# tspooner/rl_markets

Measured on AMD Instinct MI355X. Metric: env-steps/sec (whole node) at 65 536 parallel books, higher is better.
Workload: dtype f64

## Files before the change

rl_markets_amd/csrc/lob_engine.hip:

```cpp
#define LOB_TU_SPLIT 1
#define LOB_TU_MAIN 1
#include <hip/hip_runtime.h>
#include <math.h>
#include <stdio.h>
#include <stdlib.h>
#include <string.h>

#include <algorithm>
#include <climits>
#include <initializer_list>
#include <string>
#include <vector>

#include "lob_internal.h"
#include "lob_fast.h"
#include "lob_kernels.h"
#include "lob_launch.h"

#include "lob_engine_impl.h"

namespace {

void make_rndseq(uint32_t* t) {
    const int total = 344 + 4 * 2048;
// ... 114 lines not shown
            float ms = 0;
            hipEventElapsedTime(&ms, pr.first, pr.second);
            kv.second.total_ms += ms;
            kv.second.launches++;
            e->event_pool.push_back(pr.first);
            e->event_pool.push_back(pr.second);
        }
        kv.second.pending.clear();
    }
}

int device_error_rc(i32 flag) {
    if (flag) {
        std::string m = "device reported a condition on which the reference throws:";
        if (flag & LOB_ERR_BAD_ORDER_PRICE) m += " [order price <= 0]";
        if (flag & LOB_ERR_BAD_LEVEL) m += " [level price/volume <= 0]";
        if (flag & LOB_ERR_UNDEF_PRICE) m += " [undefined book price]";
        if (flag & LOB_ERR_TRADE_OVERFLOW) m += " [more trade price levels in one event than max_trades]";
        if (flag & LOB_ERR_TRACK_UNDERRUN) m += " [market-track ring underrun: raise LOB_TRACK_RING or lower LOB_TRACK_REFILL]";
        lob_set_error(m);
        return LOB_EDATA;
    }
    return LOB_OK;
}
int check_device_errors(lob_engine* e) {
    i32 flag = 0;
    HIPCHK(hipMemcpyAsync(&flag, e->S.error_flag, sizeof flag, hipMemcpyDeviceToHost, e->stream));
    HIPCHK(hipStreamSynchronize(e->stream));
    return device_error_rc(flag);
}

int finalize_episode(lob_engine* e) {
    if (!e->episode_open) return LOB_OK;
    lobk_finalize(e->stream, e->P.T <= 2, (const DevParams*)e->P_dev, e->S);
    HIPCHK(hipGetLastError());
    HIPCHK(hipStreamSynchronize(e->stream));
    e->episode_open = false;
    return LOB_OK;
}

void launch_env(lob_engine* e, hipStream_t st, const i32* actions, int count_updates, int b0, int nb, int par) {
    lobk_env(st, e->plan.env_lanes, e->P.T <= 2, (const DevParams*)e->P_dev, e->S, actions, count_updates, b0, nb, e->step_id, par);
}
void maybe_refill_track(lob_engine* e) {
    if (!e->chunked || ++e->steps_since_fill < e->sw.track_refill) return;
    e->steps_since_fill = 0;
    TimedLaunch t(e, "prepass_extend_kernel", nullptr, true);
    lobk_prepass_extend(e->stream, e->P.T <= 2, e->sw.prepass_roles, (const DevParams*)e->P_dev, e->S);
}
void launch_memo(lob_engine* e, int par, int which, int reset_lpar) {
    TimedLaunch t(e, "memo_kernel");
    hipLaunchKernelGGL(memo_kernel, dim3(256), dim3(256), 0, e->stream, e->P, e->S, (const uint32_t*)e->rnd_dev, par, which, (u64)e->theta_ver, reset_lpar);
}

void launch_step_log(lob_engine* e) {
    if (!e->slog_armed) return;
    TimedLaunch t(e, "step_log_kernel");
    StepLogSrc s;
    s.done = e->S.done; s.time_ms = e->S.time_ms; s.rec_cur = e->S.rec_cur; s.last_action = e->S.last_action;
    s.ask_level = e->S.ask_level; s.bid_level = e->S.bid_level; s.total_ticks = e->S.total_ticks;
    s.position = e->S.position;
    s.ask_quote = e->S.ask_quote; s.bid_quote = e->S.bid_quote; s.pnl_step = e->S.pnl_step;
    s.ep_pnl = e->S.ep_pnl; s.ep_bandh = e->S.ep_bandh; s.ep_reward = e->S.ep_reward;
    s.records = e->S.records; s.rec_phase = e->S.rec_phase;
    s.n_events = e->S.n_events; s.Wd = e->P.Wd; s.w_ask0 = drec_ask_px(e->P.D, e->P.T); s.w_bid0 = drec_bid_px(e->P.D, e->P.T);
    s.sel = e->slog_sel; s.n_sel = e->slog_n; s.cap = e->slog_cap;
    s.rows = e->slog_rows; s.n_rows = e->slog_cnt; s.n_lost = e->slog_cnt + e->slog_n;
    lobk_step_log(e->stream, s);
}
// ... 122 lines not shown
    P.epi_epoch = 0;
    P.seed = p->seed; P.book_id_offset = p->book_id_offset;
    P.exp_learn_first = e->sw.exp_learn_first ? 1 : 0;

    DevState& S = e->S;
    memset(&S, 0, sizeof S);
    const size_t B = (size_t)n_books;
    S.B = n_books; S.D = P.D; S.T = P.T; S.W = P.W;
    int rc = LOB_OK;
    auto alloc = [&](auto* ptr, size_t count) { if (rc == LOB_OK) rc = dev_alloc(e, ptr, count); };
#define X(t, n) alloc(&S.n, B);
    LOB_ENV_FIELDS(X)
#undef X
    alloc(&S.hdr, B);
    auto alloc_rm = [&](RMPtrs& r, int w) {
        r.w = w;
        alloc(&r.ring, B * w); alloc(&r.cnt, B); alloc(&r.head, B); alloc(&r.sum, B); alloc(&r.mean, B); alloc(&r.s, B);
    };
    auto alloc_acc = [&](AccPtrs& r, int w) {
        r.w = w;
        alloc(&r.ring, B * w); alloc(&r.cnt, B); alloc(&r.head, B); alloc(&r.sum, B);
    };
    alloc_rm(S.f_midprice, p->lb_mpm);
    alloc_rm(S.f_volatility, p->lb_vlt);
    alloc_rm(S.f_ask_tx, p->lb_svl);
    alloc_rm(S.f_bid_tx, p->lb_svl);
    alloc_rm(S.spread_window, p->lb_spread);
    alloc_rm(S.pnl_ups, p->lb_pnl);
    alloc_rm(S.pnl_downs, p->lb_pnl);
    alloc_rm(S.tp_mp, p->lb_target);
    alloc_acc(S.f_vwap_numer, p->lb_vwap);
    alloc_acc(S.f_vwap_denom, p->lb_vwap);
    alloc(&S.meta, B); alloc(&S.prep, B); alloc(&S.ewma_up, B); alloc(&S.ewma_down, B); alloc(&S.tp_val, B); alloc(&S.persist, B * LOB_PERSIST_N);
    alloc(&S.k_stop, B); alloc(&S.vars, B * 3 * 16); alloc(&S.qs_last, B * LOB_N_ACTIONS); alloc(&S.tr_idx, B * (size_t)P.trace_gens * 32);
    alloc(&S.tr_alive, B * (size_t)P.trace_gens); alloc(&S.theta, (size_t)P.M * (P.theta_private ? B : 1));
    alloc(&S.theta_nz, LOB_NZ_NWORDS(P.M) * (P.theta_private ? B : 1));
    if (P.algo == LOB_ALGO_DOUBLE_Q) {
        alloc(&S.theta_b, (size_t)P.M * (P.theta_private ? B : 1)); alloc(&S.theta_b_nz, LOB_NZ_NWORDS(P.M) * (P.theta_private ? B : 1));
        alloc(&S.qs_last_b, B * LOB_N_ACTIONS); alloc(&S.mt_state, B * LOB_MT_N); alloc(&S.mt_idx, B);
    }
    {
        const bool rl = P.r_learn != 0;
        const size_t nr = rl ? (P.theta_private ? B : 1) : 1;
        alloc(&S.rho, nr); alloc(&S.rho_inc, nr); alloc(&S.rho_cnt, nr); alloc(&S.rl_t, rl ? B : 1);
    }
    alloc(&S.tr_sig, B * (size_t)P.trace_gens * 4); alloc(&S.tr_cbslot, B * (size_t)P.trace_gens);
    {
        int slots = 2048;
        while ((size_t)slots < 8 * B && slots < (1 << 22)) slots <<= 1;
        if (e->sw.cb_slots) slots = e->sw.cb_slots;
        S.cb_slots = slots;
        alloc(&S.cb_key, (size_t)slots); alloc(&S.cb_ident, (size_t)slots * 8);
        S.cb_reps = e->sw.acc_reps ? e->sw.acc_reps : P.memo ? 8 : 1;
        alloc(&S.cb_acc, (size_t)S.cb_reps * slots * 2); alloc(&S.cb_touch, (size_t)slots); alloc(&S.cb_list, 2 * (size_t)slots);
        S.cb_segs = std::min(2048, slots / 4);
        alloc(&S.cb_count, 2 * (size_t)S.cb_segs);
        if (rc == LOB_OK && hipMemsetAsync(S.cb_key, 0xff, (size_t)slots * 8, e->stream) != hipSuccess) rc = LOB_EHIP;
        if (e->plan.dense_ids) {
            alloc(&S.cb_dense, (size_t)slots); alloc(&S.cb_free, (size_t)LOB_CBD_CAP); alloc(&S.cb_free_n, 16);
            alloc(&S.tr_cbd, B * (size_t)P.trace_gens); alloc(&S.cb_part, (size_t)LOB_ACD_MAX_BLOCKS * LOB_CBD_CAP);
            alloc(&S.cb_red, (size_t)LOB_ACD_GROUPS * LOB_CBD_CAP);
            if (rc == LOB_OK && hipMemsetAsync(S.cb_dense, 0xff, (size_t)slots * 4, e->stream) != hipSuccess) rc = LOB_EHIP;
            if (rc == LOB_OK && hipMemsetAsync(S.tr_cbd, 0xff, B * (size_t)P.trace_gens * 8, e->stream) != hipSuccess) rc = LOB_EHIP;
            if (rc == LOB_OK) {
                std::vector<i32> fl(LOB_CBD_CAP), fn(16);
                const int per = LOB_CBD_CAP / 8;
                int have = per;
// ... 1105 lines not shown
```

rl_markets_amd/csrc/lob_engine_impl.h:

```cpp
#ifndef LOB_ENGINE_IMPL_H
#define LOB_ENGINE_IMPL_H

#include <hip/hip_runtime.h>
#include <string.h>

#include <map>
#include <string>
#include <thread>
#include <utility>
#include <vector>

#include "lob_internal.h"
#include "lob_kernels.h"
#include "lob_launch.h"
#include "lob_devbuf.h"

#define HIPCHK(expr)                                                                         \
    do {                                                                                     \
        hipError_t _e = (expr);                                                              \
        if (_e != hipSuccess) {                                                              \
            lob_set_error(std::string(#expr) + ": " + hipGetErrorString(_e));                \
            return LOB_EHIP;                                                                 \
        }                                                                                    \
    } while (0)
// ... 42 lines not shown
    int groups = 1;
    bool combine = false, memo = false, carry_verdicts = false, sarsa_lanes = false;
    bool q_lanes = false;
    bool q_pair = false;
    bool t_light = false;
    bool fuse = false;
    bool fused_act_ok = false;
    bool env_step = false, half_waves = false, env16 = false;
    bool inline_ok = false;
    int env_lanes = 64;
    bool acc_block_ok = false;
    bool dense_ids = false;
    bool acc_fuse_ok = false;
    bool rest_side_ok = false;
    bool learn_first = false;
};

struct lob_engine {
    int device = 0;
    int B = 0;
    lob_params params;
    Switches sw;
    EnginePlan plan;
    DevParams P;
    DevParams* P_dev = nullptr;
    DevState S;
    DevState* S_dev = nullptr;
    DevState S_pushed;
    hipStream_t stream = nullptr;
    hipStream_t stream2 = nullptr;
    hipEvent_t ev_fork = nullptr, ev_join = nullptr, ev_stagger = nullptr;
    hipEvent_t ev_rest_go = nullptr, ev_rest_done = nullptr;
    long long flow[8] = {0, 0, 0, 0, 0, 0, 0, 0};
    long long hint_reads = 0, hint_misses = 0;
    bool dense_ever = false;
    u64* rest_hint = nullptr;
    u64* rest_hint_dev = nullptr;
    hipEvent_t hint_ev[LOB_HINT_RING] = {};
    long long hint_step = 0;
    unsigned long long hint_serial = 0;
    uint32_t hint_tags[LOB_HINT_RING] = {};
    int hint_now = 0;
    int rest_recent = 0;
    int reg_apar = 0;
    int td_parity = 0;
    int step_id = 0;
    int list_par = 0;
    int last_par = 0;
    int n_cus = 256;
    bool chunked = false;
    int steps_since_fill = 0;
    uint64_t theta_ver = 1;
    bool half_open = false;
    bool hits_ok = false;
    int steps_on_lists = 0;
    std::vector<void*> allocs;
    lob::DevBuf<uint32_t> spx_gather;
    int spx_world = 0;
    uint32_t* spx_union = nullptr;
    i32* spx_block_cnt = nullptr;
    i64* spx_block_off = nullptr;
    i64* spx_total = nullptr;
    f64* spx_buf = nullptr;
    int64_t spx_cap = 0, spx_count = 0;
    i64* spx_total_host = nullptr;
    hipEvent_t spx_ev = nullptr;
// ... 150 lines not shown
```

rl_markets_amd/csrc/lob_env.h:

```cpp
#ifndef LOB_ENV_H
#define LOB_ENV_H

#include <hip/hip_runtime.h>

#include "lob_internal.h"
#include "lob_state.h"

LOB_HD int drec_pad4(int n) { return (n + 3) & ~3; }
LOB_HD int drec_words(int D, int T) { return 4 + 4 * drec_pad4(D) + drec_pad4(2 * T); }
LOB_HD int drec_ask_px(int, int) { return 4; }
LOB_HD int drec_ask_vol(int D, int) { return 4 + drec_pad4(D); }
LOB_HD int drec_bid_px(int D, int) { return 4 + 2 * drec_pad4(D); }
LOB_HD int drec_bid_vol(int D, int) { return 4 + 3 * drec_pad4(D); }
LOB_HD int drec_trades(int D, int) { return 4 + 4 * drec_pad4(D); }
LOB_HD void drec_from_abi(const uint32_t* src, int D, int T, uint32_t* dst) {
    const int Wd = drec_words(D, T);
    for (int i = 0; i < Wd; i++) dst[i] = 0;
    dst[0] = src[LOB_REC_TIME];
    dst[1] = src[LOB_REC_FLAGS];
    for (int l = 0; l < D; l++) {
        dst[drec_ask_px(D, T) + l] = src[lob_rec_ask_px(D, T) + l];
        dst[drec_ask_vol(D, T) + l] = src[lob_rec_ask_vol(D, T) + l];
        dst[drec_bid_px(D, T) + l] = src[lob_rec_bid_px(D, T) + l];
        dst[drec_bid_vol(D, T) + l] = src[lob_rec_bid_vol(D, T) + l];
// ... 1462 lines not shown
            const f64 lm = (m.lap0 + m.lbp0) / 2.0;
            valid = ((m.ap0 - m.bp0) >= 0.0) && (mp > 0.0) && (fabs(mp - lm) < mp);
        }
        if (valid) break;
    }
    return true;
}

__device__ inline void persist_io(const DevState& S, int b, bool save) {
    int i = 0;
    const int B = S.B;
#define X(n)                                                                                   \
    if (save) { S.persist[(size_t)(i + 0) * B + b] = S.n.sum[b]; S.persist[(size_t)(i + 1) * B + b] = S.n.mean[b]; S.persist[(size_t)(i + 2) * B + b] = S.n.s[b]; } \
    else { S.n.sum[b] = S.persist[(size_t)(i + 0) * B + b]; S.n.mean[b] = S.persist[(size_t)(i + 1) * B + b]; S.n.s[b] = S.persist[(size_t)(i + 2) * B + b]; }   \
    i += 3;
    X(f_midprice) X(f_volatility) X(f_ask_tx) X(f_bid_tx) X(spread_window) X(tp_mp)
#undef X
#define X(n)                                                            \
    if (save) S.persist[(size_t)i * B + b] = S.n.sum[b];                \
    else S.n.sum[b] = S.persist[(size_t)i * B + b];                     \
    i += 1;
    X(f_vwap_numer) X(f_vwap_denom)
#undef X
    if (save) {
        S.persist[(size_t)(i + 0) * B + b] = S.ewma_up[b];
        S.persist[(size_t)(i + 1) * B + b] = S.ewma_down[b];
        S.persist[(size_t)(i + 2) * B + b] = S.tp_val[b];
    } else {
        S.ewma_up[b] = S.persist[(size_t)(i + 0) * B + b];
        S.ewma_down[b] = S.persist[(size_t)(i + 1) * B + b];
        S.tp_val[b] = S.persist[(size_t)(i + 2) * B + b];
    }
}

__device__ inline void prepass_begin(const EnvCtx& c, PrepState& st, BookMeta& M) {
    const DevParams& P = c.P;
    const DevState& S = c.S;
    const int b = c.b;
    MarketR m;
    m.cursor = 0; m.time_ms = 0; m.rec_cur = -1; m.rec_last = -1;
    m.ap0 = m.bp0 = m.lap0 = m.lbp0 = 0.0;
    m.a_tv = m.b_tv = 0;
    m.a_obsval = m.b_obsval = 0.0; m.a_obsvol = m.b_obsvol = 0;
    m.ewma_up = S.ewma_up[b]; m.ewma_down = S.ewma_down[b]; m.tp_val = S.tp_val[b];
    m.records = 0;
#define X(n) S.n.cnt[b] = 0;
    LOB_ROLLING_MEANS(X)
    LOB_ACCUMULATORS(X)
#undef X
    M.n_track = 0; M.k_warm = -1; M.init_ok = 0; M.complete = 0; M._pad = 0;
    M.ex_first = -1; M.ex_cur = -1; M.ex_last = -1; M.ex_time = 0; M.ex_records = 0;
    bool ok = true;
    while (ok && !is_open(P, m.time_ms)) ok = mk_update_book_profiles(c, m);
    M.rec_cur0 = m.rec_cur; M.rec_last0 = m.rec_last; M.time0 = m.time_ms;
    M.mid0 = (m.ap0 + m.bp0) / 2.0; M.mid_prev0 = (m.lap0 + m.lbp0) / 2.0;
    if (!ok) { M.ex_cur = m.rec_cur; M.ex_last = m.rec_last; M.ex_time = m.time_ms; M.complete = 1; }
    st.cursor = m.cursor; st.time_ms = m.time_ms; st.rec_cur = m.rec_cur; st.rec_last = m.rec_last;
    st.ap0 = m.ap0; st.bp0 = m.bp0; st.lap0 = m.lap0; st.lbp0 = m.lbp0;
    st.a_tv = m.a_tv; st.b_tv = m.b_tv;
    st.ewma_up = m.ewma_up; st.ewma_down = m.ewma_down; st.tp_val = m.tp_val;
    st.records = m.records;
    st.k = 0;
    st.prev_first = m.rec_cur;
}

__device__ inline void prepass_begin_books(const EnvCtx& c, PrepState& st, BookMeta& M) {
    const DevParams& P = c.P;
    MarketR m;
    m.cursor = 0; m.time_ms = 0; m.rec_cur = -1; m.rec_last = -1;
    m.ap0 = m.bp0 = m.lap0 = m.lbp0 = 0.0;
    m.a_tv = m.b_tv = 0;
    m.a_obsval = m.b_obsval = 0.0; m.a_obsvol = m.b_obsvol = 0;
    m.ewma_up = m.ewma_down = m.tp_val = 0.0;
    m.records = 0;
    M.n_track = 0; M.k_warm = -1; M.init_ok = 0; M.complete = 0; M._pad = 0;
    M.ex_first = -1; M.ex_cur = -1; M.ex_last = -1; M.ex_time = 0; M.ex_records = 0;
    bool ok = true;
    while (ok && !is_open(P, m.time_ms)) ok = mk_update_book_profiles(c, m);
    M.rec_cur0 = m.rec_cur; M.rec_last0 = m.rec_last; M.time0 = m.time_ms;
    M.mid0 = (m.ap0 + m.bp0) / 2.0; M.mid_prev0 = (m.lap0 + m.lbp0) / 2.0;
    if (!ok) { M.ex_cur = m.rec_cur; M.ex_last = m.rec_last; M.ex_time = m.time_ms; M.complete = 1; }
    st.cursor = m.cursor; st.time_ms = m.time_ms; st.rec_cur = m.rec_cur; st.rec_last = m.rec_last;
    st.ap0 = m.ap0; st.bp0 = m.bp0; st.lap0 = m.lap0; st.lbp0 = m.lbp0;
    st.a_tv = m.a_tv; st.b_tv = m.b_tv;
    st.ewma_up = st.ewma_down = st.tp_val = 0.0;
    st.records = m.records;
    st.k = 0;
    st.prev_first = m.rec_cur;
}

template <int TM>
__device__ inline void prepass_run(const EnvCtx& c, PrepState& st, BookMeta& M, int k_stop, bool write_track) {
    const DevParams& P = c.P;
    const DevState& S = c.S;
    const int b = c.b, B = S.B;
    MarketR m;
    m.cursor = st.cursor; m.time_ms = st.time_ms; m.rec_cur = st.rec_cur; m.rec_last = st.rec_last;
    m.ap0 = st.ap0; m.bp0 = st.bp0; m.lap0 = st.lap0; m.lbp0 = st.lbp0;
    m.a_tv = st.a_tv; m.b_tv = st.b_tv;
    m.a_obsval = m.b_obsval = 0.0; m.a_obsvol = m.b_obsvol = 0;
    m.ewma_up = st.ewma_up; m.ewma_down = st.ewma_down; m.tp_val = st.tp_val;
    m.records = st.records;
    int k = st.k;
    int prev_first = st.prev_first;
    RMReg w_mid, w_vol, w_spr, w_tp, w_atx, w_btx;
    AccReg w_vn, w_vd;
    rm_load(S.f_midprice, b, w_mid); rm_load(S.f_volatility, b, w_vol); rm_load(S.spread_window, b, w_spr);
    rm_load(S.tp_mp, b, w_tp); rm_load(S.f_ask_tx, b, w_atx); rm_load(S.f_bid_tx, b, w_btx);
    acc_load(S.f_vwap_numer, b, w_vn); acc_load(S.f_vwap_denom, b, w_vd);
#ifndef LOB_PRE_TOUCH
#define LOB_PRE_TOUCH 0
#endif
#if LOB_PRE_TOUCH
    PreRow<TM> R0;
    uint32_t nt[4] = {0u, 0u, 0u, 0u};
#else
    PreRow<TM> R0, R1;
#endif
    i32 t1 = 0, t2 = 0;
    bool piped = false;
    int band_px = 0, band_tk = 0;
    rm_prep(S.f_midprice, B, b, w_mid); rm_prep(S.f_volatility, B, b, w_vol); rm_prep(S.spread_window, B, b, w_spr);
    rm_prep(S.tp_mp, B, b, w_tp); rm_prep(S.f_ask_tx, B, b, w_atx); rm_prep(S.f_bid_tx, B, b, w_btx);
// ... 109 lines not shown
            }
            {
                f64 v_a = (f64)m.a_tv, v_b = (f64)m.b_tv;
                t.mv[LOB_MV_IMB] = (f32)((v_a + v_b) > 0 ? 5 * (v_b - v_a) / (v_b + v_a) : 0.0);
                f64 q_a = w_atx.sum, q_b = w_btx.sum;
                t.mv[LOB_MV_SVL] = (f32)((q_a + q_b) > 0 ? 5 * (q_b - q_a) / (q_a + q_b) : 0.0);
            }
            {
                f64 var = w_vol.s / (f64)(w_vol.cnt - 1);
                f64 sd = var > 0 ? sqrt(var) : 0.0;
                t.mv[LOB_MV_VOL] = (f32)ulb(5.0 * sd, 0.0, 10.0);
                f64 u = m.ewma_up, d = m.ewma_down;
                t.mv[LOB_MV_RSI] = (f32)((u + d) != 0.0 ? 5.0 * (u - d) / (u + d) : 0.0);
                f64 vw = w_vn.sum / w_vd.sum;
                t.mv[LOB_MV_VWAP] = (f32)ulb(vw / w_spr.mean, -10.0, 10.0);
                t.mv[7] = 0.0f;
            }
            c.track_w(k) = t;
            if (M.k_warm < 0 && w_atx.cnt == S.f_ask_tx.w && w_btx.cnt == S.f_bid_tx.w && w_vn.cnt == S.f_vwap_numer.w &&
                w_vd.cnt == S.f_vwap_denom.w && w_vol.cnt == S.f_volatility.w && w_mid.cnt == S.f_midprice.w &&
                w_tp.cnt == S.tp_mp.w && w_spr.cnt == S.spread_window.w)
                M.k_warm = k + 1;
        }
        if (k + 1 == M.k_warm) prev_first = m.rec_cur;
        k++;
        piped = m.cursor == first + 1;
#if LOB_PRE_TOUCH
        t2 = (i32)nt[0];
        asm volatile("" ::"v"(nt[1]), "v"(nt[2]), "v"(nt[3]));
        if (piped) t1 = t2;
#else
        if (piped) { R0 = R1; t1 = t2; }
#endif
    }
    rm_store(S.f_midprice, b, w_mid); rm_store(S.f_volatility, b, w_vol); rm_store(S.spread_window, b, w_spr);
    rm_store(S.tp_mp, b, w_tp); rm_store(S.f_ask_tx, b, w_atx); rm_store(S.f_bid_tx, b, w_btx);
    acc_store(S.f_vwap_numer, b, w_vn); acc_store(S.f_vwap_denom, b, w_vd);
    st.cursor = m.cursor; st.time_ms = m.time_ms; st.rec_cur = m.rec_cur; st.rec_last = m.rec_last;
    st.ap0 = m.ap0; st.bp0 = m.bp0; st.lap0 = m.lap0; st.lbp0 = m.lbp0;
    st.a_tv = m.a_tv; st.b_tv = m.b_tv;
    st.ewma_up = m.ewma_up; st.ewma_down = m.ewma_down; st.tp_val = m.tp_val;
    st.records = m.records;
    st.k = k;
    st.prev_first = prev_first;
    S.ewma_up[b] = m.ewma_up; S.ewma_down[b] = m.ewma_down; S.tp_val[b] = m.tp_val;
    if (write_track) {
        M.n_track = k;
        M.init_ok = M.k_warm > 0 ? 1 : 0;
    }
}


__device__ inline void lds_block_barrier() {
    __builtin_amdgcn_fence(__ATOMIC_RELEASE, "workgroup", "local");
    __builtin_amdgcn_s_barrier();
    __builtin_amdgcn_fence(__ATOMIC_ACQUIRE, "workgroup", "local");
}
struct PreXch {
    i64 mpt[64], a_obsvol[64], b_obsvol[64], a_tv[64], b_tv[64];
    f64 sp[64], mpm[64], tp_in[64], obsval[64];
    i32 spd[64], live[64];
    i32 go, _pad;
};
template <int TM>
__device__ inline void prepass_books_role(const DevParams* Pp, const DevState* Sp, int b, const uint32_t* rows, const TickLds* tk, PrepState* stp, BookMeta* Mp,
                                                int k_stop, bool on, PreXch* xch, int lane) {
    const DevParams& P = *Pp;
    const DevState& S = *Sp;
    const EnvCtx c(P, S, b, tk, rows);
    PrepState& st = *stp;
    BookMeta& M = *Mp;
    MarketR m;
    m.cursor = st.cursor; m.time_ms = st.time_ms; m.rec_cur = st.rec_cur; m.rec_last = st.rec_last;
    m.ap0 = st.ap0; m.bp0 = st.bp0; m.lap0 = st.lap0; m.lbp0 = st.lbp0;
    m.a_tv = st.a_tv; m.b_tv = st.b_tv;
    m.a_obsval = m.b_obsval = 0.0; m.a_obsvol = m.b_obsvol = 0;
    m.ewma_up = m.ewma_down = m.tp_val = 0.0;
    m.records = st.records;
    int k = st.k;
    int prev_first = st.prev_first;
    PreRow<TM> R0;
    uint32_t nt[4] = {0u, 0u, 0u, 0u};
// ... 212 lines not shown
```

rl_markets_amd/csrc/lob_kernels.h:

```cpp
#ifndef LOB_KERNELS_H
#define LOB_KERNELS_H

#include <hip/hip_runtime.h>

#include "lob_state.h"
#include "lob_stream.h"
#include "lob_launch.h"
#include "lob_stats.h"

#if !defined(LOB_TU_SPLIT)
#define LOB_IN_MAIN 1
#define LOB_IN_ENV 1
#define LOB_IN_PREPASS 1
#define LOB_IN_STATS 1
#else
#if defined(LOB_TU_STATS)
#define LOB_IN_STATS 1
#else
#define LOB_IN_STATS 0
#endif
#if defined(LOB_TU_MAIN)
#define LOB_IN_MAIN 1
#else
#define LOB_IN_MAIN 0
// ... 247 lines not shown
        f32* vf = S.vars + ((size_t)b * 3 + 2) * 16;
        const Track tk = state_track(c, e);
        for (int i = 0; i < P.V; i++) {
            v[i] = (f32)get_variable(c, e, P.vars[i], tk);
            vf[i] = v[i];
        }
        h.zero_mask &= ~(1 << last);
        S.verdict[(size_t)b * LOB_VD_STRIDE + 67] = 0;
    } else {
        e.k = M.n_track;
        e.pf = M.rec_cur0;
        e.rec_cur = M.ex_cur; e.rec_last = M.ex_last; e.time_ms = M.ex_time;
        e.mid = 0.0; e.mid_prev = 0.0;
        { const i32 n = c.n_ev(); e.events += (i64)(n > 0 ? n - 1 : 0); }
        e.done = 2;
    }
    S.hdr[b].stepped = 0;
    S.hdr[b].done = e.done;
    S.hdr[b].time_ms = e.time_ms;
    S.mk_slot[b] = -1;
    S.mk_slot_last[b] = -1;
    env_store(S, b, e);
    cnt_add(S, 1, (u64)(e.events - ev0));
}

template <int TM>
__global__ void __launch_bounds__(256, 1) finalize_kernel(const DevParams* __restrict__ Pp, DevState S) {
    const DevParams& P = *Pp;
    __shared__ TickLds tick_lds;
    stage_ticks(P, tick_lds);
    int b = blockIdx.x * blockDim.x + threadIdx.x;
    if (b >= S.B) return;
    EnvCtx c(P, S, b, &tick_lds);
    persist_io(S, b, false);
    const int k = S.k[b];
    if (k > 0) {
        PrepState st;
        BookMeta M;
        prepass_begin(c, st, M);
        M.k_warm = S.meta[b].k_warm;
        prepass_run<TM>(c, st, M, k, false);
    }
}

template <int TM>
__global__ void __launch_bounds__(64) prepass_extend_kernel(const DevParams* __restrict__ Pp, DevState S) {
    const DevParams& P = *Pp;
    __shared__ TickLds tick_lds;
    stage_ticks(P, tick_lds);
    int b = blockIdx.x * blockDim.x + threadIdx.x;
    if (b >= S.B) return;
    BookMeta M = S.meta[b];
    if (M.complete) return;
    const int k_stop = S.k[b] + S.track_len - LOB_TRACK_MARGIN;
    PrepState st = S.prep[b];
    if (st.k >= k_stop) return;
    EnvCtx c(P, S, b, &tick_lds);
    prepass_run<TM>(c, st, M, k_stop, true);
    S.meta[b] = M;
    S.prep[b] = st;
}

template <int TM>
__global__ void __launch_bounds__(128, 2) prepass_extend2_kernel(const DevParams* __restrict__ Pp, DevState S) {
    const DevParams& P = *Pp;
    __shared__ TickLds tick_lds;
    __shared__ PreXch xch[2];
    stage_ticks(P, tick_lds);
    const int role = threadIdx.x >> 6, lane = threadIdx.x & 63;
    const int t = blockIdx.x * 64 + lane;
    const bool in = t < S.B;
    const int b = in ? t : S.B - 1;
    BookMeta M = S.meta[b];
    PrepState st = S.prep[b];
    const int k_stop = S.k[b] + S.track_len - LOB_TRACK_MARGIN;
// ... 2235 lines not shown
```

rl_markets_amd/csrc/lob_state.h:

```cpp
#ifndef LOB_STATE_H
#define LOB_STATE_H

#include <stdint.h>

#include "../../include/lob_engine.h"

typedef long long i64;
typedef unsigned long long u64;
typedef int i32;
typedef double f64;
typedef float f32;

#if defined(__HIP_DEVICE_COMPILE__)
template <class T> __device__ __forceinline__ T* lob_g(T* p) {
    return (T*)(__attribute__((address_space(1))) T*)(unsigned long long)p;
}
#else
template <class T> inline T* lob_g(T* p) { return p; }
#endif

template <class T> struct GP {
    T* p;
    __host__ __device__ __forceinline__ operator T*() const { return lob_g(p); }
    __host__ __device__ __forceinline__ T* operator->() const { return lob_g(p); }
// ... 65 lines not shown
#define LOB_TRK_TRADES_OK 4
struct __attribute__((aligned(16))) TrackHead {
    i32 rec_first, rec_last, time_ms, tick_ap0;
    i32 tick_bp0, info;
    f64 mid;
};
struct __attribute__((aligned(16))) TrackHead64 {
    i32 rec_first, rec_last, time_ms, tick_ap0;
    i32 tick_bp0, info;
    f64 mid;
    f32 tr_px[2];
    f32 bap, bbp;
    i64 tr_vol[2];
};
static_assert(sizeof(TrackHead) == 32 && sizeof(TrackHead64) == 64 && sizeof(Track) == 128, "TrackHead / TrackHead64 are prefixes of Track");
#define LOB_MV_SPD 0
#define LOB_MV_MPM 1
#define LOB_MV_IMB 2
#define LOB_MV_SVL 3
#define LOB_MV_VOL 4
#define LOB_MV_RSI 5
#define LOB_MV_VWAP 6

struct BookMeta {
    i32 n_track;
    i32 k_warm;
    i32 init_ok;
    i32 rec_cur0, rec_last0, time0;
    i32 ex_first;
    i32 ex_cur, ex_last, ex_time;
    i64 ex_records;
    f64 mid0, mid_prev0;
    i32 complete;
    i32 _pad;
};

struct PrepState {
    i32 cursor, time_ms, rec_cur, rec_last;
    f64 ap0, bp0, lap0, lbp0;
    i64 a_tv, b_tv;
    f64 ewma_up, ewma_down, tp_val;
    i64 records;
    i32 k;
    i32 prev_first;
};

struct __attribute__((aligned(64))) LHdr {
    i32 done;
    i32 time_ms;
    i32 slot_cur;
    i32 zero_mask;
    i32 action;
    i32 stepped;
    i32 tr_head;
    i32 tr_n;
    u64 rng_ctr;
    f64 reward;
    f64 td;
    f64 upd;
};

#define LOB_CBD_CAP 16384
#define LOB_ACD_MAX_BLOCKS 256
#define LOB_ACD_MARK 0x7ff4000000000001ull
#define LOB_ML_BLOCKS 256
#define LOB_ML_ROWS 8192
#define LOB_PERSIST_N 32
#define LOB_PROF_N 80
#define LOB_MK_REC 10
#define LOB_MK_PROBES 16
#define LOB_HL_CAP 23
#define LOB_HL_ROW 24
#define LOB_HL_MAX 35
#define LOB_HL_REC 36
#define LOB_VD_STRIDE 72
#define LOB_NZ_SHIFT 3
#define LOB_NZ_WORD(i) ((i) >> (LOB_NZ_SHIFT + 5))
#define LOB_NZ_BIT(i) (1u << (((i) >> LOB_NZ_SHIFT) & 31))
#define LOB_NZ_NWORDS(M) ((((size_t)(M) >> LOB_NZ_SHIFT) >> 5) + 1)
#define LOB_NZ_WORDS 256
#define LOB_NZ_FILTER 128
#define LOB_NZ_NEW_MAX 256

struct RMPtrs {
    GP<f64> ring;
    GP<i32> cnt;
    GP<i32> head;
    GP<f64> sum;
    GP<f64> mean;
    GP<f64> s;
    i32 w;
};
struct AccPtrs {
    GP<f64> ring;
    GP<i32> cnt;
    GP<i32> head;
    GP<f64> sum;
    i32 w;
};

struct DevState {
    i32 B;
    i32 D, T, W;
    i32 n_events;
    GP<const uint32_t> records;
    GP<const i64> rec_phase;
    GP<const i32> rec_len;
    __device__ __forceinline__ i32 events_of(int b) const { return rec_len ? rec_len[b] : n_events; }

#define X(t, n) GP<t> n;
    LOB_ENV_FIELDS(X)
#undef X
#define X(n) RMPtrs n;
    LOB_ROLLING_MEANS(X)
#undef X
#define X(n) AccPtrs n;
    LOB_ACCUMULATORS(X)
#undef X

    GP<Track> track;
    i32 track_len, track_mask;
    GP<BookMeta> meta;
    GP<PrepState> prep;
    GP<f64> ewma_up;
    GP<f64> ewma_down;
    GP<f64> tp_val;
    GP<f64> persist;
    GP<i32> k_stop;

    GP<LHdr> hdr;
    GP<f32> vars;
    GP<f64> qs_last;
    GP<i32> tr_idx;
    GP<uint32_t> tr_alive;

    GP<f64> theta;
    GP<f64> theta_b;
    GP<uint32_t> theta_b_nz;
    GP<f64> qs_last_b;
    GP<u64> mt_state;
    GP<i32> mt_idx;
    GP<i32> tr_sig;
    GP<i32> tr_cbslot;
    GP<i32> tr_mslot;
    GP<u64> cb_key;
    GP<i32> cb_ident;
    GP<f64> cb_acc;
    GP<uint32_t> cb_touch;
    GP<i32> cb_list;
    GP<i32> cb_count;
    i32 cb_slots;
    i32 cb_reps;
    i32 cb_segs;
    i32 cb_par;
    GP<i32> cb_dense;
    GP<i32> cb_free;
    GP<i32> cb_free_n;
    GP<u64> tr_cbd;
    GP<f64> cb_part;
    GP<f64> cb_red;
    i32 cb_ids;
// ... 133 lines not shown
```

rl_markets_amd/csrc/lob_tu_host_reads.hip:

```cpp
#define LOB_TU_SPLIT 1
#include <algorithm>

#include "lob_engine_impl.h"

namespace lob {

void step_log_free(lob_engine* e) {
    if (e->slog_rows) hipFree(e->slog_rows);
    if (e->slog_cnt) hipFree(e->slog_cnt);
    if (e->slog_sel) hipFree(e->slog_sel);
    e->slog_rows = nullptr; e->slog_cnt = nullptr; e->slog_sel = nullptr;
    e->slog_n = e->slog_cap = 0;
    e->slog_armed = false;
}

}

extern "C" {

int lob_get_state(lob_engine* e, float* host_out) {
    LOB_GUARD(e, lob_get_state);
    HIPCHK(hipSetDevice(e->device));
    DevTemp<f32> d;
    if (d.alloc((size_t)e->B * e->P.V)) { lob_set_error("lob_get_state: no room for the device buffer"); return LOB_ENOMEM; }
// ... 173 lines not shown
    lobk_step_log_gather(e->stream, e->slog_rows, e->slog_cnt, e->slog_n, first_sel, n_sel, first_row, n_rows, e->slog_stage.p);
    HIPCHK(hipGetLastError());
    HIPCHK(hipMemcpyAsync(host_out, e->slog_stage.p, need * sizeof(lob_step_row), hipMemcpyDeviceToHost, e->stream));
    HIPCHK(hipStreamSynchronize(e->stream));
    return LOB_OK;
}

}

extern "C" int lob_debug_flow(lob_engine* e, int64_t out[8]) {
    if (!e || !out) return LOB_EINVAL;
    for (int i = 0; i < 8; i++) out[i] = e->flow[i];
    return LOB_OK;
}

extern "C" int lob_debug_launches(lob_engine* e, int64_t out[6]) {
    if (!e || !out) return LOB_EINVAL;
    for (int i = 0; i < 6; i++) out[i] = e->launched[i];
    return LOB_OK;
}

extern "C" int lob_debug_hint(lob_engine* e, int64_t out[2]) {
    if (!e || !out) return LOB_EINVAL;
    out[0] = e->hint_reads;
    out[1] = e->hint_misses;
    return LOB_OK;
}

extern "C" int lob_debug_exchange(lob_engine* e, int64_t out[5]) {
    if (!e || !out) return LOB_EINVAL;
    out[0] = e->spx_nosync; out[1] = e->spx_synced; out[2] = e->spx_overflows; out[3] = e->spx_fixed; out[4] = e->spx_last_total;
    return LOB_OK;
}
```

rl_markets_amd/engine.py:

```python
import ctypes as C

import numpy as np

from . import abi


class LobError(RuntimeError):
    def __init__(self, code, msg):
        super().__init__("lob_engine error %d: %s" % (code, msg))
        self.code = code


def _ptr(a):
    return a.ctypes.data_as(C.c_void_p)


def default_params():
    lib = abi.load()
    p = abi.Params()
    lib.lob_default_params(C.byref(p))
    return p


def default_gen_params():
# ... 367 lines not shown
    def counters(self):
        c = np.zeros(4, np.int64)
        self._check(self.lib.lob_get_counters(self.h, _ptr(c)))
        return c

    def path_stats(self):
        c = np.zeros(8, np.int64)
        self._check(self.lib.lob_get_path_stats(self.h, _ptr(c)))
        return c

    def flow_stats(self):
        c = np.zeros(8, np.int64)
        fn = self.lib.lob_debug_flow
        fn.restype, fn.argtypes = C.c_int, [C.c_void_p, C.c_void_p]
        self._check(fn(self.h, _ptr(c)))
        return {"added_in_place": int(c[0]), "rest_on_side_stream": int(c[1]), "block_sums": int(c[2]), "every_book": int(c[3]),
                "act_inline_general": int(c[4]), "act_work_list_dense": int(c[5]), "act_work_list_other": int(c[6]),
                "dense_sums": int(c[7])}

    def launches(self):
        c = np.zeros(6, np.int64)
        fn = self.lib.lob_debug_launches
        fn.restype, fn.argtypes = C.c_int, [C.c_void_p, C.c_void_p]
        self._check(fn(self.h, _ptr(c)))
        return {"env_step_kernel": int(c[0]), "env_step16_kernel": int(c[1]), "env_kernel_fused": int(c[2]),
                "learn_q_pair_kernel": int(c[3]), "learn_q_lane_kernel": int(c[4]), "learn_q_fast_kernel": int(c[5])}

    def hint_stats(self):
        c = np.zeros(2, np.int64)
        fn = self.lib.lob_debug_hint
        fn.restype, fn.argtypes = C.c_int, [C.c_void_p, C.c_void_p]
        self._check(fn(self.h, _ptr(c)))
        return {"hint_read": int(c[0]), "hint_missed": int(c[1])}

    def deferred_generations(self):
        c = np.zeros(1, np.int64)
        fn = self.lib.lob_debug_deferred
        fn.restype, fn.argtypes = C.c_int, [C.c_void_p, C.c_void_p]
        self._check(fn(self.h, _ptr(c)))
        return int(c[0])

    def fastpath_stats(self):
        n = 4 + 257
        c = np.zeros(n, np.int64)
        fn = self.lib.lob_debug_fastpath
        fn.restype, fn.argtypes = C.c_int, [C.c_void_p, C.c_void_p, C.c_int32]
        self._check(fn(self.h, _ptr(c), n))
        hist = c[4:]
        with_list = int(hist.sum())
        cum = np.cumsum(hist)
        def pct(q):
            return int(np.searchsorted(cum, q * with_list)) if with_list else None
        return {"written_weights": int(c[0]), "live_books": int(c[1]), "books_without_list": int(c[2]),
                "list_len_mean": round(float(c[3]) / with_list, 2) if with_list else None,
                "list_len_p50": pct(0.5), "list_len_p99": pct(0.99), "list_len_max": int(np.nonzero(hist)[0].max()) if with_list else None,
                "hist": hist}

    def fold_maps(self):
        M = int(self.M)
        words, mstride = M // 32 + 1, 2 * ((M + 1) // 2)
        nzx, nzd = np.zeros(words, np.uint32), np.zeros((2, words), np.uint32)
        nzm, terms = np.zeros((2, mstride), np.uint16), np.zeros((2, 9), np.uint32)
        fn = self.lib.lob_debug_fold_maps
        fn.restype, fn.argtypes = C.c_int, [C.c_void_p] * 5
        self._check(fn(self.h, _ptr(nzx), _ptr(nzd), _ptr(nzm), _ptr(terms)))
        return {"exact": nzx, "folded": nzd, "masks": nzm[:, :M], "terms": terms}
# ... 49 lines not shown
```

Baseline: 298.3 million.

## Checkpoint rolling-mean state in prepass so finalize skips replaying books

During the prepass, each book now saves a snapshot of its rolling-window and EWMA state (23 doubles) at the step where the market closes or the track completes, and records that step index in BookMeta. The finalize kernel restores this snapshot when the book's stop index matches it, instead of rerunning the whole prepass replay up to k. Books that do not match still fall back to the replay, and a device counter of replayed books is copied back to the host for diagnostics. The cost is extra global-memory stores inside the hot prepass loop, a per-book checkpoint buffer, and an extra memset and D2H copy at each episode end.

```diff
diff --git a/rl_markets_amd/csrc/lob_engine.hip b/rl_markets_amd/csrc/lob_engine.hip
--- a/rl_markets_amd/csrc/lob_engine.hip
+++ b/rl_markets_amd/csrc/lob_engine.hip
@@ -170,9 +170,15 @@
 
 int finalize_episode(lob_engine* e) {
     if (!e->episode_open) return LOB_OK;
+    HIPCHK(hipMemsetAsync(e->S.fin_replayed, 0, sizeof(i32), e->stream));
     lobk_finalize(e->stream, e->P.T <= 2, (const DevParams*)e->P_dev, e->S);
     HIPCHK(hipGetLastError());
-    HIPCHK(hipStreamSynchronize(e->stream));
+    i32 replayed = 0;
+    HIPCHK(hipMemcpyAsync(&replayed, e->S.fin_replayed, sizeof replayed, hipMemcpyDeviceToHost, e->stream));
+    HIPCHK(hipStreamSynchronize(e->stream));
+    e->fin_replayed = replayed;
+    e->fin_replayed_total += replayed;
+    e->fin_calls++;
     e->episode_open = false;
     return LOB_OK;
 }
@@ -361,7 +367,7 @@
     alloc_acc(S.f_vwap_numer, p->lb_vwap);
     alloc_acc(S.f_vwap_denom, p->lb_vwap);
     alloc(&S.meta, B); alloc(&S.prep, B); alloc(&S.ewma_up, B); alloc(&S.ewma_down, B); alloc(&S.tp_val, B); alloc(&S.persist, B * LOB_PERSIST_N);
-    alloc(&S.k_stop, B); alloc(&S.vars, B * 3 * 16); alloc(&S.qs_last, B * LOB_N_ACTIONS); alloc(&S.tr_idx, B * (size_t)P.trace_gens * 32);
+    alloc(&S.k_stop, B); alloc(&S.ckpt, B * LOB_CKPT_N); alloc(&S.fin_replayed, 1); alloc(&S.vars, B * 3 * 16); alloc(&S.qs_last, B * LOB_N_ACTIONS); alloc(&S.tr_idx, B * (size_t)P.trace_gens * 32);
     alloc(&S.tr_alive, B * (size_t)P.trace_gens); alloc(&S.theta, (size_t)P.M * (P.theta_private ? B : 1));
     alloc(&S.theta_nz, LOB_NZ_NWORDS(P.M) * (P.theta_private ? B : 1));
     if (P.algo == LOB_ALGO_DOUBLE_Q) {
diff --git a/rl_markets_amd/csrc/lob_engine_impl.h b/rl_markets_amd/csrc/lob_engine_impl.h
--- a/rl_markets_amd/csrc/lob_engine_impl.h
+++ b/rl_markets_amd/csrc/lob_engine_impl.h
@@ -98,6 +98,7 @@
     hipEvent_t ev_fork = nullptr, ev_join = nullptr, ev_stagger = nullptr;
     hipEvent_t ev_rest_go = nullptr, ev_rest_done = nullptr;
     long long flow[8] = {0, 0, 0, 0, 0, 0, 0, 0};
+    long long fin_replayed = 0, fin_replayed_total = 0, fin_calls = 0;
     long long hint_reads = 0, hint_misses = 0;
     bool dense_ever = false;
     u64* rest_hint = nullptr;
diff --git a/rl_markets_amd/csrc/lob_env.h b/rl_markets_amd/csrc/lob_env.h
--- a/rl_markets_amd/csrc/lob_env.h
+++ b/rl_markets_amd/csrc/lob_env.h
@@ -1518,6 +1518,19 @@
         S.tp_val[b] = S.persist[(size_t)(i + 2) * B + b];
     }
 }
+__device__ inline void ckpt_restore(const DevState& S, int b) {
+    int i = 0;
+    const int B = S.B;
+#define X(n) S.n.sum[b] = S.ckpt[(size_t)(i + 0) * B + b]; S.n.mean[b] = S.ckpt[(size_t)(i + 1) * B + b]; S.n.s[b] = S.ckpt[(size_t)(i + 2) * B + b]; i += 3;
+    X(f_midprice) X(f_volatility) X(f_ask_tx) X(f_bid_tx) X(spread_window) X(tp_mp)
+#undef X
+#define X(n) S.n.sum[b] = S.ckpt[(size_t)i * B + b]; i += 1;
+    X(f_vwap_numer) X(f_vwap_denom)
+#undef X
+    S.ewma_up[b] = S.ckpt[(size_t)(i + 0) * B + b];
+    S.ewma_down[b] = S.ckpt[(size_t)(i + 1) * B + b];
+    S.tp_val[b] = S.ckpt[(size_t)(i + 2) * B + b];
+}
 
 __device__ inline void prepass_begin(const EnvCtx& c, PrepState& st, BookMeta& M) {
     const DevParams& P = c.P;
@@ -1534,7 +1547,7 @@
     LOB_ROLLING_MEANS(X)
     LOB_ACCUMULATORS(X)
 #undef X
-    M.n_track = 0; M.k_warm = -1; M.init_ok = 0; M.complete = 0; M._pad = 0;
+    M.n_track = 0; M.k_warm = -1; M.init_ok = 0; M.complete = 0; M.k_ckpt = -1;
     M.ex_first = -1; M.ex_cur = -1; M.ex_last = -1; M.ex_time = 0; M.ex_records = 0;
     bool ok = true;
     while (ok && !is_open(P, m.time_ms)) ok = mk_update_book_profiles(c, m);
@@ -1559,7 +1572,7 @@
     m.a_obsval = m.b_obsval = 0.0; m.a_obsvol = m.b_obsvol = 0;
     m.ewma_up = m.ewma_down = m.tp_val = 0.0;
     m.records = 0;
-    M.n_track = 0; M.k_warm = -1; M.init_ok = 0; M.complete = 0; M._pad = 0;
+    M.n_track = 0; M.k_warm = -1; M.init_ok = 0; M.complete = 0; M.k_ckpt = -1;
     M.ex_first = -1; M.ex_cur = -1; M.ex_last = -1; M.ex_time = 0; M.ex_records = 0;
     bool ok = true;
     while (ok && !is_open(P, m.time_ms)) ok = mk_update_book_profiles(c, m);
@@ -1575,6 +1588,20 @@
     st.prev_first = m.rec_cur;
 }
 
+#if defined(__HIP_DEVICE_COMPILE__)
+#define LOB_CKPT_PIN(x, y) asm volatile("" : "+v"(x), "+s"(y))
+#else
+#define LOB_CKPT_PIN(x, y) ((void)0)
+#endif
+#define LOB_CKPT_STORE() do { int i = 0; size_t cb = (size_t)b; int cB = B; LOB_CKPT_PIN(cb, cB); \
+        S.ckpt[(size_t)(i++) * cB + cb] = w_mid.sum; S.ckpt[(size_t)(i++) * cB + cb] = w_mid.mean; S.ckpt[(size_t)(i++) * cB + cb] = w_mid.s; \
+        S.ckpt[(size_t)(i++) * cB + cb] = w_vol.sum; S.ckpt[(size_t)(i++) * cB + cb] = w_vol.mean; S.ckpt[(size_t)(i++) * cB + cb] = w_vol.s; \
+        S.ckpt[(size_t)(i++) * cB + cb] = w_atx.sum; S.ckpt[(size_t)(i++) * cB + cb] = w_atx.mean; S.ckpt[(size_t)(i++) * cB + cb] = w_atx.s; \
+        S.ckpt[(size_t)(i++) * cB + cb] = w_btx.sum; S.ckpt[(size_t)(i++) * cB + cb] = w_btx.mean; S.ckpt[(size_t)(i++) * cB + cb] = w_btx.s; \
+        S.ckpt[(size_t)(i++) * cB + cb] = w_spr.sum; S.ckpt[(size_t)(i++) * cB + cb] = w_spr.mean; S.ckpt[(size_t)(i++) * cB + cb] = w_spr.s; \
+        S.ckpt[(size_t)(i++) * cB + cb] = w_tp.sum; S.ckpt[(size_t)(i++) * cB + cb] = w_tp.mean; S.ckpt[(size_t)(i++) * cB + cb] = w_tp.s; \
+        S.ckpt[(size_t)(i++) * cB + cb] = w_vn.sum; S.ckpt[(size_t)(i++) * cB + cb] = w_vd.sum; \
+        S.ckpt[(size_t)(i++) * cB + cb] = m.ewma_up; S.ckpt[(size_t)(i++) * cB + cb] = m.ewma_down; S.ckpt[(size_t)(i++) * cB + cb] = m.tp_val; } while (0)
 template <int TM>
 __device__ inline void prepass_run(const EnvCtx& c, PrepState& st, BookMeta& M, int k_stop, bool write_track) {
     const DevParams& P = c.P;
@@ -1750,7 +1777,11 @@
 #else
         if (piped) { R0 = R1; t1 = t2; }
 #endif
-    }
+        if (write_track && M.k_ckpt < 0 && M.k_warm > 0 && !is_open(P, m.time_ms)) { M.k_ckpt = k; LOB_CKPT_STORE(); }
+    }
+    if (write_track && M.k_ckpt < 0 && M.complete) { M.k_ckpt = k; LOB_CKPT_STORE(); }
+#undef LOB_CKPT_STORE
+#undef LOB_CKPT_PIN
     rm_store(S.f_midprice, b, w_mid); rm_store(S.f_volatility, b, w_vol); rm_store(S.spread_window, b, w_spr);
     rm_store(S.tp_mp, b, w_tp); rm_store(S.f_ask_tx, b, w_atx); rm_store(S.f_bid_tx, b, w_btx);
     acc_store(S.f_vwap_numer, b, w_vn); acc_store(S.f_vwap_denom, b, w_vd);
@@ -1766,6 +1797,22 @@
         M.n_track = k;
         M.init_ok = M.k_warm > 0 ? 1 : 0;
     }
+}
+
+template <int TM>
+__device__ inline bool finalize_book(const EnvCtx& c, int k) {
+    const DevState& S = c.S;
+    const int b = c.b;
+    if (k == S.meta[b].k_ckpt) { ckpt_restore(S, b); return false; }
+    persist_io(S, b, false);
+    if (k > 0) {
+        PrepState st;
+        BookMeta M;
+        prepass_begin(c, st, M);
+        M.k_warm = S.meta[b].k_warm;
+        prepass_run<TM>(c, st, M, k, false);
+    }
+    return true;
 }
 
 
diff --git a/rl_markets_amd/csrc/lob_kernels.h b/rl_markets_amd/csrc/lob_kernels.h
--- a/rl_markets_amd/csrc/lob_kernels.h
+++ b/rl_markets_amd/csrc/lob_kernels.h
@@ -303,15 +303,7 @@
     int b = blockIdx.x * blockDim.x + threadIdx.x;
     if (b >= S.B) return;
     EnvCtx c(P, S, b, &tick_lds);
-    persist_io(S, b, false);
-    const int k = S.k[b];
-    if (k > 0) {
-        PrepState st;
-        BookMeta M;
-        prepass_begin(c, st, M);
-        M.k_warm = S.meta[b].k_warm;
-        prepass_run<TM>(c, st, M, k, false);
-    }
+    if (finalize_book<TM>(c, S.k[b])) atomicAdd((i32*)S.fin_replayed, 1);
 }
 
 template <int TM>
diff --git a/rl_markets_amd/csrc/lob_state.h b/rl_markets_amd/csrc/lob_state.h
--- a/rl_markets_amd/csrc/lob_state.h
+++ b/rl_markets_amd/csrc/lob_state.h
@@ -121,7 +121,7 @@
     i64 ex_records;
     f64 mid0, mid_prev0;
     i32 complete;
-    i32 _pad;
+    i32 k_ckpt;
 };
 
 struct PrepState {
@@ -155,6 +155,7 @@
 #define LOB_ML_BLOCKS 256
 #define LOB_ML_ROWS 8192
 #define LOB_PERSIST_N 32
+#define LOB_CKPT_N 23
 #define LOB_PROF_N 80
 #define LOB_MK_REC 10
 #define LOB_MK_PROBES 16
@@ -216,6 +217,8 @@
     GP<f64> tp_val;
     GP<f64> persist;
     GP<i32> k_stop;
+    GP<f64> ckpt;
+    GP<i32> fin_replayed;
 
     GP<LHdr> hdr;
     GP<f32> vars;
diff --git a/rl_markets_amd/csrc/lob_tu_host_reads.hip b/rl_markets_amd/csrc/lob_tu_host_reads.hip
--- a/rl_markets_amd/csrc/lob_tu_host_reads.hip
+++ b/rl_markets_amd/csrc/lob_tu_host_reads.hip
@@ -229,3 +229,9 @@
     out[0] = e->spx_nosync; out[1] = e->spx_synced; out[2] = e->spx_overflows; out[3] = e->spx_fixed; out[4] = e->spx_last_total;
     return LOB_OK;
 }
+
+extern "C" int lob_debug_finalize(lob_engine* e, int64_t out[3]) {
+    if (!e || !out) return LOB_EINVAL;
+    out[0] = e->fin_replayed; out[1] = e->fin_replayed_total; out[2] = e->fin_calls;
+    return LOB_OK;
+}
diff --git a/rl_markets_amd/engine.py b/rl_markets_amd/engine.py
--- a/rl_markets_amd/engine.py
+++ b/rl_markets_amd/engine.py
@@ -423,6 +423,13 @@
         fn.restype, fn.argtypes = C.c_int, [C.c_void_p, C.c_void_p]
         self._check(fn(self.h, _ptr(c)))
         return {"hint_read": int(c[0]), "hint_missed": int(c[1])}
+
+    def finalize_stats(self):
+        c = np.zeros(3, np.int64)
+        fn = self.lib.lob_debug_finalize
+        fn.restype, fn.argtypes = C.c_int, [C.c_void_p, C.c_void_p]
+        self._check(fn(self.h, _ptr(c)))
+        return {"replayed_last": int(c[0]), "replayed_total": int(c[1]), "episode_ends": int(c[2])}
 
     def deferred_generations(self):
         c = np.zeros(1, np.int64)
```

Result: no change. 300.0 million (median of 6 runs) (+0.6%).
